# haowenz/FEM

Measured on AMD Instinct MI355X. Metric: mapped Mreads/s (100 bp, e=3) at 1/2/4/8 MI355X + achieved HBM GB/s vs roofline, higher is better.
Workload: dtype u32/u64 integer + 32-bit Myers bit-vectors

## Files before the change

fem_amd/csrc/fem_hip.hip:

```cpp
#include "../../include/fem_hip.h"

#include <hip/hip_runtime.h>
#include <rccl/rccl.h>
#include <sched.h>
#if defined(__x86_64__)
#include <immintrin.h>
#endif

#include <algorithm>
#include <cctype>
#include <cstdio>
#include <cstdlib>
#include <cstring>
#include <condition_variable>
#include <functional>
#include <atomic>
#include <chrono>
#include <mutex>
#include <string>
#include <thread>
#include <vector>

#include "fem_index_build.hip.h"
#include "fem_pack.h"
// ... 476 lines not shown
  hipFuncAttributes a{};
  const bool banked = which == 1;
  const void *f = join ? (const void *)join_kernel(R, which)
                       : banked ? (const void *)femk::seed_select_kernel<R, true> : (const void *)femk::seed_select_kernel<R>;
  return hipFuncGetAttributes(&a, f) == hipSuccess && a.numRegs > 0 ? (uint32_t)a.numRegs : 128u;
}
uint32_t kernel_regs(int R, bool join, int which = 0) {
  static std::atomic<uint32_t> cache[3][2][femk::kMaxR + 1] = {};
  std::atomic<uint32_t> &slot = cache[which][join ? 1 : 0][std::min(std::max(R, 1), femk::kMaxR)];
  uint32_t c = slot.load(std::memory_order_relaxed);
  if (c) return c;
#define FEM_CALL(r) c = kernel_regs_r<r>(join, which)
  FEM_DENSE_SWITCH(R, FEM_CALL)
#undef FEM_CALL
  slot.store(c, std::memory_order_relaxed);
  return c;
}
int select_blocks_per_cu(int R, bool banked, int block, uint32_t lds) {
  int nb = 0;
#define FEM_CALL(r) nb = select_blocks_per_cu_r<r>(banked, block, lds)
  FEM_DENSE_SWITCH(R, FEM_CALL)
#undef FEM_CALL
  return nb;
}
void launch_select(int R, bool banked, dim3 grid, dim3 block, uint32_t lds, hipStream_t st, const femk::SeedParams &sp) {
#define FEM_CALL(r) launch_select_r<r>(banked, grid, block, lds, st, sp)
  FEM_DENSE_SWITCH(R, FEM_CALL)
#undef FEM_CALL
}
int join_blocks_per_cu(int R, int which, int block, uint32_t lds) {
  int nb = 0;
  return hipOccupancyMaxActiveBlocksPerMultiprocessor(&nb, join_kernel(R, which), block, lds) == hipSuccess ? nb : 0;
}
void launch_join(int R, int which, dim3 grid, dim3 block, uint32_t lds, hipStream_t st, const femk::SeedParams &sp) {
  hipLaunchKernelGGL(join_kernel(R, which), grid, block, lds, st, sp);
}

template <int R>
void launch_fast(bool hash, dim3 grid, dim3 block, uint32_t lds, hipStream_t st, const femk::SeedParams &sp) {
  if (hash)
    hipLaunchKernelGGL((femk::seed_fast_kernel<R, true>), grid, block, lds, st, sp);
  else
    hipLaunchKernelGGL((femk::seed_fast_kernel<R, false>), grid, block, lds, st, sp);
}

template <int R>
int fast_blocks_per_cu_r(bool hash, int block, uint32_t lds) {
  int nb = 0;
  hipError_t err = hash ? hipOccupancyMaxActiveBlocksPerMultiprocessor(&nb, femk::seed_fast_kernel<R, true>, block, lds)
                        : hipOccupancyMaxActiveBlocksPerMultiprocessor(&nb, femk::seed_fast_kernel<R, false>, block, lds);
  return err == hipSuccess ? nb : 0;
}
int fast_blocks_per_cu(int R, bool hash, int block, uint32_t lds) {
  switch (R) {
    case 1: return fast_blocks_per_cu_r<1>(hash, block, lds);
    case 2: return fast_blocks_per_cu_r<2>(hash, block, lds);
    case 3: return fast_blocks_per_cu_r<3>(hash, block, lds);
    case 4: return fast_blocks_per_cu_r<4>(hash, block, lds);
    case 5: return fast_blocks_per_cu_r<5>(hash, block, lds);
    case 6: return fast_blocks_per_cu_r<6>(hash, block, lds);
    case 7: return fast_blocks_per_cu_r<7>(hash, block, lds);
    case 8: return fast_blocks_per_cu_r<8>(hash, block, lds);
    case 9: return fast_blocks_per_cu_r<9>(hash, block, lds);
    default: return fast_blocks_per_cu_r<10>(hash, block, lds);
  }
}

// ... 729 lines not shown
  }
  if (!ok_ev) {
    (void)fem_dev_close(h);
    return FEM_ERR_HIP;
  }
  if (testing_switch("FEM_TESTING")) {
    h->no_overlap = testing_switch("FEM_NO_OVERLAP");
    h->no_parts = testing_switch("FEM_NO_PARTS");
    if (const char *mp = getenv("FEM_PARTS")) h->max_parts = std::min(kMaxParts, std::max(1, atoi(mp)));
    h->timeline = testing_switch("FEM_TIMELINE");
    if (h->timeline && hipEventCreate(&h->ev_epoch) == hipSuccess && hipEventRecord(h->ev_epoch, h->side_stream) == hipSuccess)
      h->timing = true, h->have_epoch = true;
    h->force_generic = testing_switch("FEM_FORCE_GENERIC");
    h->force_hash = testing_switch("FEM_FORCE_HASH");
    h->force_dense = testing_switch("FEM_FORCE_DENSE");
    h->no_dense = testing_switch("FEM_NO_DENSE");
    h->no_strided = testing_switch("FEM_NO_STRIDED");
    h->tiny_buffers = testing_switch("FEM_TEST_TINY_BUFFERS");
    if (const char *bl = getenv("FEM_TEST_BANK_BASES")) h->bank_limit = strtoull(bl, nullptr, 10);
    if (const char *bs = getenv("FEM_TEST_BANK_SEQS")) h->bank_seqs = (uint32_t)strtoul(bs, nullptr, 10);
  }
  *out = h;
  return FEM_OK;
}

int fem_dev_close(fem_dev *h) {
  if (!h) return FEM_ERR_INVALID;
  {
    std::lock_guard<std::mutex> lock(g_comm_mu);
    if (g_comm && std::find(g_comm->devs.begin(), g_comm->devs.end(), h->device) != g_comm->devs.end()) destroy_comm_set();
  }
  (void)hipSetDevice(h->device);
  (void)hipDeviceSynchronize();
  delete h->stage_pool;
  h->stage_pool = nullptr;
  for (auto &s : h->slot) {
    drain_timing(h, s);
    for (void *p : {(void *)s.d_bases_alloc, (void *)s.d_off, (void *)s.d_cand, (void *)s.d_meta, (void *)s.d_ed,
                    (void *)s.d_end, (void *)s.d_begin, (void *)s.d_count, (void *)s.d_nmap, (void *)s.d_ctl,
                    (void *)s.d_arena, (void *)s.d_slow, (void *)s.d_sel, (void *)s.d_sel_hdr, (void *)s.d_packed, (void *)s.d_exc_bits, (void *)s.d_quals, (void *)s.d_names,
                    (void *)s.d_name_off, (void *)s.d_count8, (void *)s.d_seg, (void *)s.d_pcand, (void *)s.d_ped, (void *)s.d_pend, (void *)s.d_big})
      if (p) (void)hipFree(p);
    for (void *p : {(void *)s.h_ctl, (void *)s.h_begin, (void *)s.h_count, (void *)s.h_cand, (void *)s.h_ed,
                    (void *)s.h_end, (void *)s.h_bases, (void *)s.h_off, (void *)s.h_quals, (void *)s.h_names, (void *)s.h_name_off,
                    (void *)s.h_count8, (void *)s.h_seg, (void *)s.h_pcand, (void *)s.h_ped, (void *)s.h_pend, (void *)s.h_big})
      if (p) (void)hipHostFree(p);
    if (s.stream) (void)hipStreamDestroy(s.stream);
    if (s.text_stream) (void)hipStreamDestroy(s.text_stream);
    if (s.out_stream) (void)hipStreamDestroy(s.out_stream);
    if (s.ev_text_staged) (void)hipEventDestroy(s.ev_text_staged);
    if (s.ev_text_order) (void)hipEventDestroy(s.ev_text_order);
    delete s.tail;
    s.tail = nullptr;
  }
  delete h->bgzf;
  h->bgzf = nullptr;
  if (h->d_zin) (void)hipFree(h->d_zin);
  if (h->z_stream) (void)hipStreamDestroy(h->z_stream);
  if (h->d_ref_names) (void)hipFree(h->d_ref_names);
  if (h->d_ref_name_off) (void)hipFree(h->d_ref_name_off);
  for (hipEvent_t e : h->event_pool) (void)hipEventDestroy(e);
  if (h->ev_kernels_done) (void)hipEventDestroy(h->ev_kernels_done);
  if (h->ev_select_done) (void)hipEventDestroy(h->ev_select_done);
  if (h->ev_h2d_done) (void)hipEventDestroy(h->ev_h2d_done);
  if (h->ev_epoch) (void)hipEventDestroy(h->ev_epoch);
  if (h->side_stream) (void)hipStreamDestroy(h->side_stream);
// ... 1259 lines not shown
```

fem_amd/csrc/fem_host.cc:

```cpp
#include "fem_host.h"
#include "fem_pack.h"

#include <fcntl.h>
#include <omp.h>
#include <sys/mman.h>
#include <sys/stat.h>
#include <unistd.h>
#include <zlib.h>
#if defined(__x86_64__)
#include <immintrin.h>
#endif

#include <algorithm>
#include <cctype>
#include <cstdio>
#include <cstdlib>
#include <cstring>
#include <condition_variable>
#include <functional>
#include <mutex>
#include <string>
#include <thread>
#include <vector>

namespace {
class SleepingPool {
 public:
  ~SleepingPool() {
    {
      std::lock_guard<std::mutex> l(mu_);
      stop_ = true;
    }
    cv_.notify_all();
    for (auto &t : threads_) t.join();
// ... 2141 lines not shown
    buf.push_back('\n');
    buf.push_back('+');
    buf.push_back('\n');
    buf.insert(buf.end(), qual.begin(), qual.end());
    buf.push_back('\n');
    if (buf.size() > (1u << 24) - 1024) {
      if (fwrite(buf.data(), 1, buf.size(), f) != buf.size()) {
        fclose(f);
        return -2;
      }
      buf.clear();
    }
  }
  bool ok = fwrite(buf.data(), 1, buf.size(), f) == buf.size();
  return (fclose(f) == 0 && ok) ? 0 : -2;
}

int fem_synth_write_fasta(const char *path, const char *text, const uint64_t *seq_off, const uint32_t *seq_len,
                          uint32_t n_seq) {
  FILE *f = fopen(path, "wb");
  if (!f) return -1;
  bool ok = true;
  for (uint32_t s = 0; s < n_seq && ok; ++s) {
    ok = fprintf(f, ">chr%u synthetic\n", s + 1) > 0;
    const char *p = text + seq_off[s];
    for (uint64_t i = 0; i < seq_len[s] && ok; i += 60) {
      size_t n = (size_t)std::min<uint64_t>(60, seq_len[s] - i);
      ok = fwrite(p + i, 1, n, f) == n && fputc('\n', f) != EOF;
    }
  }
  return (fclose(f) == 0 && ok) ? 0 : -2;
}

}
```

fem_amd/csrc/fem_host.h:

```cpp
#ifndef FEM_HOST_H_
#define FEM_HOST_H_

#include <stddef.h>
#include <stdint.h>

#ifdef __cplusplus
extern "C" {
#endif

typedef struct fem_seqfile fem_seqfile;

typedef struct {
  uint64_t n;
  char *bases;
  uint64_t *off;
  char *quals;
  char *names;
  uint64_t *name_off;
} fem_seqset;

fem_seqfile *fem_seqfile_open(const char *path);
void fem_seqfile_close(fem_seqfile *f);
int fem_seqfile_read(fem_seqfile *f, uint64_t max_seqs, fem_seqset *out);
int fem_seqfile_read_bytes(fem_seqfile *f, uint64_t approx_bytes, int n_threads, fem_seqset *out);
// ... 78 lines not shown
  const uint32_t *md_off;
  const char *md;
} fem_record_view;
int fem_records_sam(const fem_tail_ref *ref, const fem_seqset *reads, const fem_record_view *rec, int n_threads,
                    char **text, uint64_t *text_len);
typedef struct {
  uint64_t offset, length;
} fem_text_part;
int fem_records_sam_parts(const fem_tail_ref *ref, const fem_seqset *reads, const fem_record_view *rec, int n_threads,
                          char **buf, uint64_t *cap, fem_text_part *parts, uint64_t *n_asserted);
int fem_records_sam_refs(const fem_tail_ref *ref, const fem_read_refs *reads, const fem_record_view *rec, int n_threads, char **buf,
                         uint64_t *cap, fem_text_part *parts, uint64_t *n_asserted);
int fem_sam_header(const fem_tail_ref *ref, char **text, uint64_t *text_len);
int fem_bam_header(const fem_tail_ref *ref, uint8_t **raw, uint64_t *len);
int fem_sam_fill_quals(char *text, uint64_t text_len, const uint64_t *qual_at, uint64_t n_reads, const char *quals, const uint64_t *off,
                       uint32_t read_len, int n_threads);

void fem_synth_reference(uint64_t seed, uint32_t n_seq, const uint64_t *seq_off, const uint32_t *seq_len, char *out,
                         int n_threads);
void fem_synth_reads(uint64_t seed, const char *ref_text, const uint64_t *seq_off, const uint32_t *seq_len,
                     uint32_t n_seq, uint64_t first_read, uint64_t n_reads, uint32_t L, int32_t e, char *bases_out,
                     int n_threads);
void fem_synth_reads_ex(uint64_t seed, const char *ref_text, const uint64_t *seq_off, const uint32_t *seq_len,
                        uint32_t n_seq, uint64_t first_read, uint64_t n_reads, uint32_t L, int32_t e, char *bases_out,
                        uint8_t *n_err_out, int n_threads);

void fem_synth_reads_packed(uint64_t seed, const char *ref_text, const uint64_t *seq_off, const uint32_t *seq_len, uint32_t n_seq,
                            uint64_t first_read, uint64_t n_reads, uint32_t L, int32_t e, uint8_t *codes, int n_threads);

int fem_synth_write_fastq(const char *path, const char *bases, uint32_t L, uint64_t n_reads, uint64_t first_index);
int fem_synth_write_fasta(const char *path, const char *text, const uint64_t *seq_off, const uint32_t *seq_len,
                          uint32_t n_seq);

#ifdef __cplusplus
}
#endif
#endif
```

fem_amd/csrc/fem_kernels.hip.h:

```cpp
#pragma once
#include <hip/hip_runtime.h>
#include <stdint.h>
#include "fem_planes.hip.h"

namespace femk {

constexpr int kWave = 64;
constexpr uint32_t kFlagCandOverflow = 1u;
constexpr uint32_t kFlagArenaOverflow = 2u;
constexpr uint32_t kFlagTooLarge = 4u;
constexpr uint32_t kInvalidMeta = 0xFFFFFFFFu;
constexpr int kMaxR = 10;
constexpr uint32_t kMeta16 = 0x80000000u;
constexpr uint32_t kSlotChunk = 256u;
constexpr uint32_t kFlagQueueOverflow = 8u;
constexpr uint32_t kQueueChunk = 32u;
constexpr uint32_t kInvalidRead = 0xFFFFFFFFu;

struct SeedLayout {
  uint32_t pkw, nkw;
  uint32_t sf;
  uint32_t dp_rows;
  uint32_t dp_bits;
  uint32_t picked;
// ... 18 lines not shown
  uint32_t *work_cursor;
  const uint32_t *lookup;
  const uint64_t *occ;
  uint32_t inf32;
  const uint32_t *seq_len;
  int32_t e, a, R, k, step, lg;
  uint64_t *cand;
  uint32_t *cand_meta;
  uint32_t cand_cap;
  uint32_t *cand_begin;
  uint32_t *cand_count;
  uint32_t *ctr;
  uint32_t n_seq;
  uint32_t *slow_queue;
  uint32_t slow_cap;
  const uint32_t *work_queue;
  const uint32_t *summary;
  const uint32_t *occ32;
  uint32_t list_shift;
  const uint32_t *goff;
  const uint32_t *blkseq;
  const uint32_t *freq11;
  uint2 *sel;
  uint2 *sel_hdr;
  uint32_t n_banks;
  uint32_t bank_first[5];
  const uint32_t *bank_lo;
  uint32_t n_buckets;
  uint32_t blk_stride;
  unsigned long long *stats;
  uint64_t *arena;
  unsigned long long arena_cap;
  unsigned long long *arena_ctr;
  SeedLayout lay;
};

__global__ void uniform_offsets_kernel(uint64_t *off, uint64_t n, uint32_t len) {
  const uint64_t stride = (uint64_t)gridDim.x * blockDim.x;
  for (uint64_t i = (uint64_t)blockIdx.x * blockDim.x + threadIdx.x; i <= n; i += stride) off[i] = i * (uint64_t)len;
}

__global__ void unpack_reads_kernel(const uint8_t *packed, uint64_t n_reads, uint32_t len, uint32_t bytes_per_read, uint8_t *bases) {
  const uint64_t stride = (uint64_t)gridDim.x * blockDim.x, total = n_reads * bytes_per_read;
  const bool aligned = (len & 3u) == 0u && (((uintptr_t)bases) & 3u) == 0u;
  for (uint64_t i = (uint64_t)blockIdx.x * blockDim.x + threadIdx.x; i < total; i += stride) {
    const uint32_t b = packed[i];
    const uint32_t c0 = (0x54474341u >> (8u * (b & 3u))) & 0xFFu, c1 = (0x54474341u >> (8u * ((b >> 2) & 3u))) & 0xFFu;
    const uint32_t c2 = (0x54474341u >> (8u * ((b >> 4) & 3u))) & 0xFFu, c3 = (0x54474341u >> (8u * (b >> 6))) & 0xFFu;
    if (aligned) {
      ((uint32_t *)bases)[i] = c0 | (c1 << 8) | (c2 << 16) | (c3 << 24);
    } else {
      const uint64_t r = i / bytes_per_read;
      const uint32_t k = (uint32_t)(i - r * bytes_per_read) * 4u;
      uint8_t *o = bases + r * len + k;
      o[0] = (uint8_t)c0;
      if (k + 1u < len) o[1] = (uint8_t)c1;
      if (k + 2u < len) o[2] = (uint8_t)c2;
      if (k + 3u < len) o[3] = (uint8_t)c3;
    }
  }
}
__global__ void scatter_chars_kernel(const uint32_t *at, const uint8_t *ch, uint64_t n, uint8_t *bases) {
  const uint64_t stride = (uint64_t)gridDim.x * blockDim.x;
  for (uint64_t i = (uint64_t)blockIdx.x * blockDim.x + threadIdx.x; i < n; i += stride) bases[at[i]] = ch[i];
}

// ... 1347 lines not shown
```

fem_amd/csrc/fem_seed_join.hip.h:

```cpp
#pragma once
#include "fem_seed_dense.hip.h"

namespace femk {

#ifndef FEM_JOIN_SLOTS_HI
#define FEM_JOIN_SLOTS_HI 32768u
#endif
#ifndef FEM_JOIN_OPT
#define FEM_JOIN_OPT 15
#endif
#ifndef FEM_JOIN_OPT_HI
#define FEM_JOIN_OPT_HI 12
#endif
#ifndef FEM_JOIN_ABL
#define FEM_JOIN_ABL 0
#endif
#ifndef FEM_JOIN_SLOTS_LO
#define FEM_JOIN_SLOTS_LO 32768u
#endif
constexpr uint32_t join_slots(int R, bool padded = false) { return R >= 7 ? FEM_JOIN_SLOTS_HI : padded ? FEM_JOIN_SLOTS_LO : 32768u; }
#ifndef FEM_JOIN_BATCH_HI
#define FEM_JOIN_BATCH_HI 3
#endif

constexpr uint32_t join_bitmap_words(int R, bool padded = false) { return join_slots(R, padded) / 32u + 4u; }

__device__ __forceinline__ void lds_or(uint32_t *w, uint32_t bits) {
  (void)__hip_atomic_fetch_or(w, bits, __ATOMIC_RELAXED, __HIP_MEMORY_SCOPE_WAVEFRONT);
}

template <int R, bool BANKED = false, bool PADDED = false>
__device__ bool join_read(const SeedParams &p, uint32_t s_start, uint32_t s_lo, uint32_t s_freq, uint32_t *bitmap,
                          uint32_t *flg , uint32_t *scatter ,
                          uint32_t *cand_lds, uint32_t &kept0, uint32_t &kept1, uint32_t seq_base = 0u ) {
// ... 441 lines not shown
          const uint32_t fv = ln < nfl ? flg[gg * kFlgStride + ln] : 0u;
          uint32_t rank = 0;
          for (uint64_t m = pm; m;) {
            const int j = __builtin_ctzll(m);
            m &= m - 1;
            const uint32_t x = (uint32_t)__builtin_amdgcn_readlane((int)fv, j);
            rank += (uint32_t)(x < fv || (x == fv && (uint32_t)j < ln));
          }
          wave_sync_lds();
          if (mine) scatter[rank] = fv;
          wave_sync_lds();
          const uint32_t fs = ln < nF ? scatter[ln] : 0u;
          kept = dense_merge_group(cv, kept, fs, nF, e);
          if (kept == 0xFFFFFFFFu) return false;
        }
      }
    }
    cand_lds[(u >= (uint32_t)kStep ? (uint32_t)kWave : 0u) + ln] = cv;
    if (u >= (uint32_t)kStep) kept1 = kept; else kept0 = kept;
    cmin = 0xFFFFFFFFu, cmax = 0u, any_hi = false;
    pm0 = pm1 = pm2 = 0, nf0 = nf1 = nf2 = 0;
  }
  return true;
}

#ifndef FEM_JOIN_WAVES_LO
#define FEM_JOIN_WAVES_LO 7
#endif
#ifndef FEM_JOIN_WAVES_HI
#define FEM_JOIN_WAVES_HI 6
#endif

constexpr int join_waves(int R) { return R <= 6 ? FEM_JOIN_WAVES_LO : FEM_JOIN_WAVES_HI; }

template <int R, bool BANKED = false, bool PADDED = false>
__device__ __forceinline__ void seed_join_body(const SeedParams &p, uint8_t *smem) {
  constexpr uint32_t kSeeds = (uint32_t)(kStep * R);
  static_assert(2 * kStep * R <= kWave, "both strands' seeds must fit the lanes of one wave");
  const uint32_t ln = lane_id();
  const uint32_t wave_in_block = (uint32_t)__builtin_amdgcn_readfirstlane((int)(threadIdx.x >> 6));
  uint8_t *wbase = smem + (size_t)wave_in_block * p.lay.wave_bytes;
  uint32_t *scatter = (uint32_t *)(wbase + p.lay.X);
  uint32_t *flg = (uint32_t *)(wbase + p.lay.A);
  uint32_t *bitmap = (uint32_t *)(wbase + p.lay.F);
  uint2 *blk_entries = (uint2 *)(wbase + p.lay.B);
  uint32_t *cand_lds = (uint32_t *)(wbase + p.lay.sf);
  uint2 *seqtab = (uint2 *)(smem + p.lay.picked);
  const bool small_ref = p.n_seq <= (uint32_t)kWave;
  if (wave_in_block == 0) seqtab[ln] = ln < p.n_seq ? make_uint2(p.goff[ln], p.seq_len[ln]) : make_uint2(0xFFFFFFFFu, 0u);
  __syncthreads();
  for (uint32_t i = ln; i < join_bitmap_words(R, PADDED); i += kWave) bitmap[i] = i < join_slots(R, PADDED) / 32u ? 0u : 0xFFFFFFFFu;
  wave_sync_lds();
  unsigned long long pre_sum = 0, cand_sum = 0;
  SlotChunk chunk, qchunk;

  auto queue_slow = [&](uint32_t read) {
    if (qchunk.left == 0) {
      uint32_t base = 0;
      if (ln == 0) base = atomicAdd(&p.ctr[2], kQueueChunk);
      qchunk.next = bcast0(base);
      qchunk.left = kQueueChunk;
    }
    if (qchunk.next < p.slow_cap) {
      if (ln == 0) p.slow_queue[qchunk.next] = read;
    } else if (ln == 0) {
      atomicOr(&p.ctr[1], kFlagQueueOverflow);
    }
    ++qchunk.next, --qchunk.left;
  };

  for (;;) {
    uint32_t pull = 0;
    if (ln == 0) pull = atomicAdd(p.work_cursor, kReadBlock);
    pull = bcast0(pull);
    if ((uint64_t)p.read_begin + pull >= p.n_reads) break;
    const uint32_t r0 = p.read_begin + pull;
    const uint32_t n_blk = p.n_reads - r0 < kReadBlock ? p.n_reads - r0 : kReadBlock;
    if (ln < 2u * kReadBlock) blk_entries[ln] = make_uint2(kBlkSkip, 0u);
    uint2 hdr = make_uint2(kSelSlow, 0u);
    if (ln < n_blk) hdr = p.sel_hdr[r0 + ln];
    uint2 sel_next = make_uint2(0u, 0u);
    if (!BANKED && ln < 2u * kSeeds) sel_next = p.sel[(size_t)r0 * (2u * kSeeds) + ln];
    for (uint32_t rb = 0; rb < n_blk; ++rb) {
      const uint32_t read = r0 + rb;
      const uint32_t h0 = (uint32_t)__builtin_amdgcn_readlane((int)hdr.x, (int)rb);
      const uint32_t status = h0 & 3u, L = h0 >> 8;
      const uint2 sel = sel_next;
      if (!BANKED && rb + 1u < n_blk && ln < 2u * kSeeds) sel_next = p.sel[(size_t)(read + 1u) * (2u * kSeeds) + ln];
      if (status == kSelSlow) continue;
      if (status == kSelNone) {
        if (ln / 2u == rb) blk_entries[ln] = make_uint2(0u, 0u);
        continue;
      }
      if constexpr (BANKED) {
        constexpr uint32_t kStash = (uint32_t)kWave;
        uint64_t *stash = (uint64_t *)(wbase + p.lay.gq);
        uint32_t acc[2] = {0u, 0u};
        bool failed = false;
        for (uint32_t b = 0; b < p.n_banks && !failed; ++b) {
          uint2 sel_b = make_uint2(0u, 0u);
          if (ln < 2u * kSeeds) sel_b = p.sel[((size_t)read * p.n_banks + b) * (2u * kSeeds) + ln];
          uint32_t kept0 = 0, kept1 = 0;
          if (!join_read<R, true>(p, sel_b.y & 0xFFFFu, sel_b.x, sel_b.y >> 16, bitmap, flg, scatter, cand_lds, kept0, kept1, p.bank_first[b])) {
            failed = true;
            break;
          }
          const uint32_t sq_lo = p.bank_first[b], sq_hi = p.bank_first[b + 1u];
#pragma unroll 1
          for (uint32_t strand = 0; strand < 2u; ++strand) {
            const uint32_t kept = strand ? kept1 : kept0;
            if (kept == 0) continue;
            const uint32_t v = cand_lds[strand * (uint32_t)kWave + ln];
            uint32_t sq = 0, pos = 0, slen = 0;
            if (small_ref) {
              const uint2 tab = seqtab[ln];
              const bool mine = ln >= sq_lo && ln < sq_hi;
              for (uint32_t i = 0; i < kept; ++i) {
                const uint32_t vi = (uint32_t)__builtin_amdgcn_readlane((int)v, (int)i);
                const uint32_t s_i = sq_lo + (uint32_t)__popcll(__builtin_amdgcn_ballot_w64(mine && tab.x <= vi)) - 1u;
                const uint32_t g_i = (uint32_t)__builtin_amdgcn_readlane((int)tab.x, (int)s_i);
                const uint32_t l_i = (uint32_t)__builtin_amdgcn_readlane((int)tab.y, (int)s_i);
                if (ln == i) sq = s_i, pos = vi - g_i, slen = l_i;
              }
            } else if (ln < kept) {
              sq = p.blkseq[(size_t)b * p.blk_stride + (v >> kDenseBlkShift)];
              while (sq + 1u < sq_hi && p.goff[sq + 1u] <= v) ++sq;
              pos = v - p.goff[sq];
              slen = p.seq_len[sq];
            }
            const bool ok = ln < kept && pos >= (uint32_t)p.e && pos + L + (uint32_t)p.e < slen;
            const uint64_t mo = __ballot(ok);
            const uint32_t n_ok = (uint32_t)__popcll(mo);
            if (acc[strand] + n_ok > kStash) {
              failed = true;
              break;
            }
            if (ok) stash[strand * kStash + acc[strand] + (uint32_t)__popcll(mo & ((1ull << ln) - 1ull))] = (((uint64_t)sq << 32) | pos) - (uint64_t)p.e;
            acc[strand] += n_ok;
          }
        }
        if (failed) {
          queue_slow(read);
          continue;
        }
        pre_sum += (uint32_t)__builtin_amdgcn_readlane((int)hdr.y, (int)rb);
        wave_sync_lds();
#pragma unroll 1
        for (uint32_t strand = 0; strand < 2u; ++strand) {
          const uint32_t n_out = acc[strand];
          uint32_t base = 0;
          if (n_out > 0) {
            if (n_out <= chunk.left) {
              base = chunk.next;
              chunk.next += n_out, chunk.left -= n_out;
            } else {
              pad_chunk(p, chunk);
              if (ln == 0) base = atomicAdd(&p.ctr[0], kSlotChunk);
              base = bcast0(base);
              chunk.next = base + n_out, chunk.left = kSlotChunk - n_out;
            }
            if ((unsigned long long)base + n_out > p.cand_cap) {
              if (ln == 0) atomicOr(&p.ctr[1], kFlagCandOverflow);
            } else {
              for (uint32_t i = ln; i < n_out; i += (uint32_t)kWave) {
                p.cand[base + i] = stash[strand * kStash + i];
                p.cand_meta[base + i] = (read * 2u + strand) | (i < (n_out & ~7u) ? kMeta16 : 0u);
              }
            }
          }
          if (ln == 0) blk_entries[2u * rb + strand] = make_uint2(base, n_out);
          cand_sum += n_out;
        }
        wave_sync_lds();
        continue;
      }
      const uint32_t s_lo = sel.x, s_start = sel.y & 0xFFFFu, s_freq = sel.y >> 16;
      uint32_t kept0 = 0, kept1 = 0;
      if (!join_read<R, false, PADDED>(p, s_start, s_lo, s_freq, bitmap, flg, scatter, cand_lds, kept0, kept1)) {
        queue_slow(read);
        continue;
      }
      if (FEM_JOIN_ABL & 16) kept0 = kept1 = 0;
      pre_sum += (uint32_t)__builtin_amdgcn_readlane((int)hdr.y, (int)rb);
#pragma unroll 1
      for (uint32_t strand = 0; strand < 2u; ++strand) {
        const uint32_t kept = strand ? kept1 : kept0;
        uint64_t out = 0;
        bool ok = false;
        if (kept == 0) {
          if (ln == 0) blk_entries[2u * rb + strand] = make_uint2(0u, 0u);
          continue;
        }
        const uint32_t v = cand_lds[strand * (uint32_t)kWave + ln];
        uint32_t sq = 0, pos = 0, slen = 0;
        if (small_ref) {
          const uint2 tab = seqtab[ln];
          for (uint32_t i = 0; i < kept; ++i) {
            const uint32_t vi = (uint32_t)__builtin_amdgcn_readlane((int)v, (int)i);
            const uint32_t s_i = (uint32_t)__popcll(__builtin_amdgcn_ballot_w64(tab.x <= vi)) - 1u;
            const uint32_t g_i = (uint32_t)__builtin_amdgcn_readlane((int)tab.x, (int)s_i);
            const uint32_t l_i = (uint32_t)__builtin_amdgcn_readlane((int)tab.y, (int)s_i);
            if (ln == i) sq = s_i, pos = vi - g_i, slen = l_i;
          }
        } else if (ln < kept) {
          sq = p.blkseq[v >> kDenseBlkShift];
          while (sq + 1u < p.n_seq && p.goff[sq + 1u] <= v) ++sq;
          pos = v - p.goff[sq];
          slen = p.seq_len[sq];
        }
        if (ln < kept) {
          ok = pos >= (uint32_t)p.e && pos + L + (uint32_t)p.e < slen;
          out = (((uint64_t)sq << 32) | pos) - (uint64_t)p.e;
        }
        const uint64_t mo = __ballot(ok);
        const uint32_t n_out = (uint32_t)__popcll(mo);
        uint32_t base = 0;
        if (n_out > 0) {
          if (n_out <= chunk.left) {
            base = chunk.next;
            chunk.next += n_out, chunk.left -= n_out;
          } else {
            pad_chunk(p, chunk);
            if (ln == 0) base = atomicAdd(&p.ctr[0], kSlotChunk);
            base = bcast0(base);
            chunk.next = base + n_out, chunk.left = kSlotChunk - n_out;
          }
          if ((unsigned long long)base + n_out > p.cand_cap) {
            if (ln == 0) atomicOr(&p.ctr[1], kFlagCandOverflow);
          } else if (ok) {
            const uint32_t rank = (uint32_t)__popcll(mo & ((1ull << ln) - 1ull)), at = base + rank;
            p.cand[at] = out;
            p.cand_meta[at] = (read * 2u + strand) | (rank < (n_out & ~7u) ? kMeta16 : 0u);
          }
        }
        if (ln == 0) blk_entries[2u * rb + strand] = make_uint2(base, n_out);
        cand_sum += n_out;
      }
    }
    wave_sync_lds();
    const uint2 entry = blk_entries[ln];
    wave_sync_lds();
    if (ln < 2u * kReadBlock && r0 + ln / 2u < p.n_reads && entry.x != kBlkSkip) {
      __builtin_nontemporal_store(entry.x, &p.cand_begin[r0 * 2u + ln]);
      __builtin_nontemporal_store(entry.y, &p.cand_count[r0 * 2u + ln]);
    }
  }
  pad_chunk(p, chunk);
  for (uint32_t i = ln; i < qchunk.left; i += kWave)
    if (qchunk.next + i < p.slow_cap) p.slow_queue[qchunk.next + i] = kInvalidRead;
  if (ln == 0) {
    if (pre_sum) atomicAdd(&p.stats[0], pre_sum);
    if (cand_sum) atomicAdd(&p.stats[1], cand_sum);
  }
}


#define FEM_JOIN_KERNEL(R, WAVES)                                                                                               \
  __global__ void __launch_bounds__(256) __attribute__((amdgpu_waves_per_eu(WAVES, 8))) seed_join_kernel_r##R(SeedParams p) {                         \
    extern __shared__ __attribute__((aligned(16))) uint8_t smem[];                                                               \
    seed_join_body<R>(p, smem);                                                                                                  \
  }                                                                                                                              \
  __global__ void __launch_bounds__(256) __attribute__((amdgpu_waves_per_eu(FEM_JOIN_WAVES_HI, 8))) seed_join_banked_kernel_r##R(SeedParams p) {  \
    extern __shared__ __attribute__((aligned(16))) uint8_t smem[];                                                               \
    seed_join_body<R, true>(p, smem);                                                                                            \
  }                                                                                                                              \
  __global__ void __launch_bounds__(256) __attribute__((amdgpu_waves_per_eu(WAVES, 8))) seed_join_kernel_padded_r##R(SeedParams p) {  \
    extern __shared__ __attribute__((aligned(16))) uint8_t smem[];                                                               \
    seed_join_body<R, false, true>(p, smem);                                                                                     \
  }
FEM_JOIN_KERNEL(1, FEM_JOIN_WAVES_LO)
FEM_JOIN_KERNEL(2, FEM_JOIN_WAVES_LO)
FEM_JOIN_KERNEL(3, FEM_JOIN_WAVES_LO)
FEM_JOIN_KERNEL(4, FEM_JOIN_WAVES_LO)
FEM_JOIN_KERNEL(5, FEM_JOIN_WAVES_LO)
FEM_JOIN_KERNEL(6, FEM_JOIN_WAVES_LO)
FEM_JOIN_KERNEL(7, FEM_JOIN_WAVES_HI)
FEM_JOIN_KERNEL(8, FEM_JOIN_WAVES_HI)
FEM_JOIN_KERNEL(9, FEM_JOIN_WAVES_HI)
FEM_JOIN_KERNEL(10, FEM_JOIN_WAVES_HI)
// ... 4 lines not shown
```

fem_amd/csrc/fem_seed_select.hip.h:

```cpp
#pragma once
#include <type_traits>

#include "fem_seed_fast.hip.h"

namespace femk {

constexpr uint32_t kDenseMaxBanks = 4;
constexpr uint32_t kDenseNear = 1024u;
constexpr uint32_t kDenseRemap = 0xF0000000u;
constexpr uint32_t kSelKeepAll = 1u << 15;
constexpr uint32_t kSelOk = 0u, kSelNone = 1u, kSelSlow = 2u;
constexpr uint32_t kSelMaxCols = 128u;
constexpr uint32_t kSelMaxList = 128u;
constexpr uint32_t kX11 = 1u << 22;

__device__ __forceinline__ uint32_t wave_min_u32(uint32_t x) {
  constexpr uint32_t kFill = 0xFFFFFFFFu;
  x = dpp_min_step<0x111, 0xF>(x, kFill), x = dpp_min_step<0x112, 0xF>(x, kFill), x = dpp_min_step<0x114, 0xF>(x, kFill);
  x = dpp_min_step<0x118, 0xF>(x, kFill), x = dpp_min_step<0x142, 0xA>(x, kFill), x = dpp_min_step<0x143, 0xC>(x, kFill);
  return (uint32_t)__builtin_amdgcn_readlane((int)x, 63);
}
__device__ __forceinline__ uint32_t wave_max_u32(uint32_t x) {
  return (uint32_t)__builtin_amdgcn_readlane((int)wave_scan_max(x), 63);
}
// ... 87 lines not shown

template <int R, bool BANKED = false>
__global__ void __launch_bounds__(256) __attribute__((amdgpu_waves_per_eu(FEM_SELECT_WAVES, 8))) seed_select_kernel(SeedParams p) {
  extern __shared__ __attribute__((aligned(16))) uint8_t smem[];
  const uint32_t ln = lane_id();
  const uint32_t wave_in_block = (uint32_t)__builtin_amdgcn_readfirstlane((int)(threadIdx.x >> 6));
  uint8_t *wbase = smem + (size_t)wave_in_block * p.lay.wave_bytes;
  uint64_t *boff = (uint64_t *)(wbase + p.lay.rb);
  uint32_t *fw = (uint32_t *)(wbase + p.lay.strm);
  uint32_t *nw = fw + p.lay.strm_words;
  uint16_t *fq = (uint16_t *)(wbase + p.lay.fq);
  uint32_t *r_base = (uint32_t *)(wbase + p.lay.rinfo), *r_len = r_base + kReadBlock, *r_flag = r_len + kReadBlock,
           *r_pre = r_flag + kReadBlock;
  constexpr uint32_t kOk0 = 1u, kOk1 = 2u, kShape = 4u, kSlow = 8u;
  const uint32_t sstride = p.lay.gstride, nb = p.lay.nb;
  const uint32_t inf = p.inf32;
  SlotChunk qchunk;

  auto queue_slow = [&](uint32_t read) {
    if (qchunk.left == 0) {
      uint32_t base = 0;
      if (ln == 0) base = atomicAdd(&p.ctr[2], kQueueChunk);
      qchunk.next = bcast0(base);
      qchunk.left = kQueueChunk;
    }
    if (qchunk.next < p.slow_cap) {
      if (ln == 0) p.slow_queue[qchunk.next] = read;
    } else if (ln == 0) {
      atomicOr(&p.ctr[1], kFlagQueueOverflow);
    }
    ++qchunk.next, --qchunk.left;
  };

  for (;;) {
    uint32_t pull = 0;
    if (ln == 0) pull = atomicAdd(p.work_cursor, kReadBlock);
    pull = bcast0(pull);
    if ((uint64_t)p.read_begin + pull >= p.n_reads) break;
    const uint32_t r0 = p.read_begin + pull;
    const uint32_t n_blk = p.n_reads - r0 < kReadBlock ? p.n_reads - r0 : kReadBlock;
    wave_sync_lds();
    if (ln <= n_blk) boff[ln] = p.read_off[r0 + ln];
    wave_sync_lds();
    for (uint32_t sb = 0; sb < n_blk; sb += nb) {
      const uint32_t cnt = n_blk - sb < nb ? n_blk - sb : nb;
      const uint32_t rd0 = r0 + sb;
      const uint64_t o_first = boff[sb];
      const uint64_t blk_off = (uint64_t)__builtin_amdgcn_readfirstlane((uint32_t)o_first) |
                               ((uint64_t)__builtin_amdgcn_readfirstlane((uint32_t)(o_first >> 32)) << 32);
      uint32_t my_S = 0, my_flag = 0;
      {
        uint32_t L = 0, base = 0;
        if (ln < cnt) {
          const uint64_t o0 = boff[sb + ln], o1 = boff[sb + ln + 1u];
          L = (uint32_t)(o1 - o0), base = (uint32_t)(o0 - blk_off);
          const int S = (int)L - kK + 1;
          bool shape_ok = S > 0 && R <= S / kStep;
          if (shape_ok) shape_ok = (S - (kStep - 1)) / kStep - R * kLg + 2 >= 2;
          if (shape_ok) {
            my_S = (uint32_t)S;
            my_flag = kShape | kOk0 | kOk1;
            const uint32_t widest = (uint32_t)(S / kStep - R * kLg + 1);
            if (widest > kSelMaxCols || p.a == 0) my_flag |= kSlow;
          }
        }
        if (ln < kReadBlock) r_base[ln] = base, r_len[ln] = L, r_flag[ln] = my_flag, r_pre[ln] = 0;
      }
      const uint32_t total_chars = (uint32_t)(boff[sb + cnt] - blk_off);
      uint32_t any_n = 0;
      {
        const uint8_t *src = p.bases + blk_off;
// ... 238 lines not shown
```

fem_amd/host.py:

```python
import ctypes as C
import os

import numpy as np

_HERE = os.path.dirname(os.path.abspath(__file__))
_LIB = None


class SeqSet(C.Structure):
    _fields_ = [("n", C.c_uint64), ("bases", C.c_void_p), ("off", C.c_void_p), ("quals", C.c_void_p),
                ("names", C.c_void_p), ("name_off", C.c_void_p)]


class TailInput(C.Structure):
    _fields_ = [("n_reads", C.c_uint64), ("cand_begin", C.c_void_p), ("cand_count", C.c_void_p), ("cand", C.c_void_p),
                ("ed", C.c_void_p), ("end", C.c_void_p)]


class TailRef(C.Structure):
    _fields_ = [("text", C.c_void_p), ("off", C.c_void_p), ("len", C.c_void_p), ("n_seq", C.c_uint32),
                ("names", C.c_void_p), ("name_off", C.c_void_p)]


class Records(C.Structure):
# ... 32 lines not shown
        L.fem_seqfile_open.restype = vp
        L.fem_seqfile_open.argtypes = [C.c_char_p]
        L.fem_seqfile_close.argtypes = [vp]
        L.fem_seqfile_read.argtypes = [vp, u64, C.POINTER(SeqSet)]
        L.fem_seqset_free.argtypes = [C.POINTER(SeqSet)]
        L.fem_seqfile_read_bytes.argtypes = [vp, u64, C.c_int, C.POINTER(SeqSet)]
        L.fem_seqfile_plan.argtypes = [vp, u64, C.c_int, C.POINTER(vp), C.POINTER(BatchShape)]
        L.fem_seqfile_plan_count.argtypes = [vp, u64, C.c_int, C.POINTER(vp), C.POINTER(BatchShape)]
        L.fem_seqfile_fill.argtypes = [vp, vp, C.c_int, vp, vp, vp, vp, vp]
        L.fem_seqfile_fill_packed.argtypes = [vp, vp, C.c_int, C.c_uint32, vp, u64, C.POINTER(u64), vp, vp, vp]
        L.fem_seqfile_fill_packed_refs.argtypes = [vp, vp, C.c_int, C.c_uint32, vp, u64, C.POINTER(u64), vp]
        L.fem_batch_plan_free.argtypes = [vp]
        L.fem_records_sam.argtypes = [C.POINTER(TailRef), C.POINTER(SeqSet), C.POINTER(RecordView), C.c_int, C.POINTER(vp),
                                      C.POINTER(u64)]
        L.fem_records_sam_parts.argtypes = [C.POINTER(TailRef), C.POINTER(SeqSet), C.POINTER(RecordView), C.c_int,
                                            C.POINTER(vp), C.POINTER(u64), C.POINTER(TextPart), C.POINTER(u64)]
        L.fem_index_save.argtypes = [C.c_char_p, i32, i32, vp, u64, vp]
        L.fem_index_load.argtypes = [C.c_char_p, C.POINTER(i32), C.POINTER(i32), C.POINTER(vp), C.POINTER(u64),
                                     C.POINTER(vp)]
        L.fem_tail_records.argtypes = [i32, C.POINTER(TailRef), vp, vp, C.POINTER(TailInput), C.c_int,
                                       C.POINTER(Records)]
        L.fem_records_free.argtypes = [C.POINTER(Records)]
        L.fem_tail_sam.argtypes = [i32, C.POINTER(TailRef), C.POINTER(SeqSet), C.POINTER(TailInput), C.c_int,
                                   C.POINTER(vp), C.POINTER(u64)]
        L.fem_sam_header.argtypes = [C.POINTER(TailRef), C.POINTER(vp), C.POINTER(u64)]
        L.fem_bam_header.argtypes = [C.POINTER(TailRef), C.POINTER(vp), C.POINTER(u64)]
        L.fem_sam_fill_quals.argtypes = [vp, u64, vp, u64, vp, vp, C.c_uint32, C.c_int]
        L.fem_synth_reference.argtypes = [u64, C.c_uint32, vp, vp, vp, C.c_int]
        L.fem_synth_reads.argtypes = [u64, vp, vp, vp, C.c_uint32, u64, u64, C.c_uint32, i32, vp, C.c_int]
        L.fem_synth_reads_ex.argtypes = [u64, vp, vp, vp, C.c_uint32, u64, u64, C.c_uint32, i32, vp, vp, C.c_int]
        L.fem_synth_reads_packed.argtypes = [u64, vp, vp, vp, C.c_uint32, u64, u64, C.c_uint32, i32, vp, C.c_int]
        L.fem_synth_write_fastq.argtypes = [C.c_char_p, vp, C.c_uint32, u64, u64]
        L.fem_synth_write_fasta.argtypes = [C.c_char_p, vp, vp, vp, C.c_uint32]
        L.free = C.CDLL(None).free
        L.free.argtypes = [vp]
        _LIB = L
    return _LIB


def _copy(ptr, n, dtype):
    n = int(n)
    if n == 0 or not ptr:
        return np.zeros(0, dtype=dtype)
    buf = (C.c_char * (n * np.dtype(dtype).itemsize)).from_address(ptr)
    return np.frombuffer(buf, dtype=dtype, count=n).copy()


def synth_reference(seed, seq_lens, threads=8):
    lens = np.asarray(seq_lens, dtype=np.uint32)
    off = np.zeros(len(lens), dtype=np.uint64)
    if len(lens) > 1:
        off[1:] = np.cumsum(lens[:-1], dtype=np.uint64)
    total = int(lens.astype(np.uint64).sum())
    text = np.zeros(total + 64, dtype=np.uint8)
    lib().fem_synth_reference(seed, len(lens), off.ctypes.data, lens.ctypes.data, text.ctypes.data, threads)
    return text, off, lens


def synth_reads(seed, text, off, lens, n_reads, L, e, first_read=0, threads=8, out=None, out_offsets=None, n_err=None):
    bases = np.zeros(n_reads * L + 8, dtype=np.uint8) if out is None else out
    assert bases.dtype == np.uint8 and len(bases) >= n_reads * L
    ne = 0
    if n_err is not None:
        assert n_err.dtype == np.uint8 and len(n_err) >= n_reads
        ne = n_err.ctypes.data
    lib().fem_synth_reads_ex(seed, text.ctypes.data, off.ctypes.data, lens.ctypes.data, len(lens), first_read, n_reads,
                             L, e, bases.ctypes.data, ne, threads)
    if out_offsets is None:
        offsets = np.arange(n_reads + 1, dtype=np.uint64) * np.uint64(L)
    else:
        offsets = out_offsets
        offsets[:n_reads + 1] = np.arange(n_reads + 1, dtype=np.uint64) * np.uint64(L)
    return bases, offsets


def synth_reads_packed(seed, text, off, lens, n_reads, L, e, out, first_read=0, threads=8):
    bpr = (L + 3) // 4
    assert out.dtype == np.uint8 and len(out) >= ((n_reads * bpr + 7) & ~7)
    lib().fem_synth_reads_packed(seed, text.ctypes.data, off.ctypes.data, lens.ctypes.data, len(lens), first_read, n_reads,
                                 L, e, out.ctypes.data, threads)
    return out


def write_fastq(path, bases, L, n_reads, first_index=0):
    rc = lib().fem_synth_write_fastq(path.encode(), bases.ctypes.data, L, n_reads, first_index)
    if rc != 0:
        raise OSError("fem_synth_write_fastq failed (%d)" % rc)


def write_fasta(path, text, off, lens):
    rc = lib().fem_synth_write_fasta(path.encode(), text.ctypes.data, off.ctypes.data, lens.ctypes.data, len(lens))
    if rc != 0:
        raise OSError("fem_synth_write_fasta failed (%d)" % rc)


class Sequences:

    def __init__(self, s):
        n = int(s.n)
        self.n = n
        self.off = _copy(s.off, n + 1, np.uint64)
        self.name_off = _copy(s.name_off, n + 1, np.uint64)
        nb = int(self.off[-1]) if n else 0
        self.bases = _copy(s.bases, nb, np.uint8)
        self.quals = _copy(s.quals, nb, np.uint8) if s.quals else None
        self.names_raw = _copy(s.names, int(self.name_off[-1]) if n else 0, np.uint8)

    def seq(self, i):
        return self.bases[int(self.off[i]):int(self.off[i + 1])].tobytes()

    def name(self, i):
        return self.names_raw[int(self.name_off[i]):int(self.name_off[i + 1])].tobytes().decode()

    def qual(self, i):
        return self.quals[int(self.off[i]):int(self.off[i + 1])].tobytes()


def read_sequences(path, max_seqs=0):
    L = lib()
    f = L.fem_seqfile_open(path.encode())
    if not f:
        raise FileNotFoundError(path)
    s = SeqSet()
    rc = L.fem_seqfile_read(f, max_seqs, C.byref(s))
    L.fem_seqfile_close(f)
    try:
# ... 348 lines not shown
```

Before: 336.8.

## Schedule join work with guided tickets, prefetch next block, and static first pull

Replaces the join kernel's fixed-size atomic read-block pulls with a ticket scheme. Blocks of 16 reads shrink to 8/4/2/1 near the tail to balance the end of the launch. The first ticket is assigned statically, and the next ticket is drawn and its headers prefetched one read before the current block ends, to hide atomic and load latency. The select kernel also gets a static first pull, and candidate slot chunks grow to fit large outputs. Optional timestamp instrumentation and host ticket helpers are added for testing, at the cost of more complex scheduling logic.

After: 320.2. -4.9%, worse.

```diff
diff --git a/fem_amd/csrc/fem_hip.hip b/fem_amd/csrc/fem_hip.hip
--- a/fem_amd/csrc/fem_hip.hip
+++ b/fem_amd/csrc/fem_hip.hip
@@ -532,7 +532,44 @@
   int nb = 0;
   return hipOccupancyMaxActiveBlocksPerMultiprocessor(&nb, join_kernel(R, which), block, lds) == hipSuccess ? nb : 0;
 }
+#ifdef FEM_JOIN_STAMPS
+constexpr uint32_t kStampLaunches = 32, kStampWaves = 16384;
+struct StampRing {
+  unsigned long long *d = nullptr;
+  uint64_t launches = 0;
+  uint64_t waves[kStampLaunches], reads[kStampLaunches];
+} g_stamps;
+unsigned long long *stamps_next(uint32_t waves, uint32_t reads) {
+  if (!g_stamps.d && hipMalloc((void **)&g_stamps.d, sizeof(unsigned long long) * 4u * kStampWaves * kStampLaunches) != hipSuccess) return nullptr;
+  if (waves > kStampWaves) return nullptr;
+  const uint32_t at = (uint32_t)(g_stamps.launches++ % kStampLaunches);
+  g_stamps.waves[at] = waves, g_stamps.reads[at] = reads;
+  return g_stamps.d + (size_t)at * 4u * kStampWaves;
+}
+void stamps_dump() {
+  if (!g_stamps.d || !g_stamps.launches) return;
+  const char *path = getenv("FEM_JOIN_STAMPS_OUT");
+  FILE *f = fopen(path ? path : "join_stamps.bin", "wb");
+  const uint64_t n = std::min<uint64_t>(g_stamps.launches, kStampLaunches);
+  std::vector<unsigned long long> buf(4u * kStampWaves);
+  for (uint64_t i = 0; f && i < n; ++i) {
+    const uint32_t at = (uint32_t)((g_stamps.launches - n + i) % kStampLaunches);
+    if (hipMemcpy(buf.data(), g_stamps.d + (size_t)at * 4u * kStampWaves, sizeof(unsigned long long) * 4u * g_stamps.waves[at], hipMemcpyDeviceToHost) != hipSuccess) break;
+    const unsigned long long head[2] = {g_stamps.waves[at], g_stamps.reads[at]};
+    fwrite(head, sizeof(head), 1, f);
+    fwrite(buf.data(), sizeof(unsigned long long), 4u * g_stamps.waves[at], f);
+  }
+  if (f) fclose(f);
+  g_stamps.launches = 0;
+}
+#endif
 void launch_join(int R, int which, dim3 grid, dim3 block, uint32_t lds, hipStream_t st, const femk::SeedParams &sp) {
+#ifdef FEM_JOIN_STAMPS
+  femk::SeedParams stamped = sp;
+  stamped.stamps = stamps_next(grid.x * (block.x / 64u), sp.n_reads - sp.read_begin);
+  hipLaunchKernelGGL(join_kernel(R, which), grid, block, lds, st, stamped);
+  return;
+#endif
   hipLaunchKernelGGL(join_kernel(R, which), grid, block, lds, st, sp);
 }
 
@@ -1328,6 +1365,9 @@
   }
   (void)hipSetDevice(h->device);
   (void)hipDeviceSynchronize();
+#ifdef FEM_JOIN_STAMPS
+  stamps_dump();
+#endif
   delete h->stage_pool;
   h->stage_pool = nullptr;
   for (auto &s : h->slot) {
diff --git a/fem_amd/csrc/fem_host.cc b/fem_amd/csrc/fem_host.cc
--- a/fem_amd/csrc/fem_host.cc
+++ b/fem_amd/csrc/fem_host.cc
@@ -1,5 +1,6 @@
 #include "fem_host.h"
 #include "fem_pack.h"
+#include "fem_ticket.h"
 
 #include <fcntl.h>
 #include <omp.h>
@@ -2207,4 +2208,17 @@
   return (fclose(f) == 0 && ok) ? 0 : -2;
 }
 
-}
+uint32_t fem_join_ticket_block(uint32_t t, uint32_t n, uint32_t waves, uint32_t *out) {
+  const femticket::Block b = femticket::block_of(t, n, waves);
+  if (out) out[0] = b.first, out[1] = b.count;
+  return femticket::ticket_count(n, waves);
+}
+uint32_t fem_join_ticket_blocks(uint32_t n, uint32_t waves, uint32_t *first, uint32_t *count, uint32_t cap) {
+  for (uint32_t t = 0; t < cap; ++t) {
+    const femticket::Block b = femticket::block_of(t, n, waves);
+    first[t] = b.first, count[t] = b.count;
+  }
+  return femticket::ticket_count(n, waves);
+}
+
+}
diff --git a/fem_amd/csrc/fem_host.h b/fem_amd/csrc/fem_host.h
--- a/fem_amd/csrc/fem_host.h
+++ b/fem_amd/csrc/fem_host.h
@@ -134,6 +134,9 @@
 int fem_synth_write_fasta(const char *path, const char *text, const uint64_t *seq_off, const uint32_t *seq_len,
                           uint32_t n_seq);
 
+uint32_t fem_join_ticket_block(uint32_t t, uint32_t n, uint32_t waves, uint32_t *out);
+uint32_t fem_join_ticket_blocks(uint32_t n, uint32_t waves, uint32_t *first, uint32_t *count, uint32_t cap);
+
 #ifdef __cplusplus
 }
 #endif
diff --git a/fem_amd/csrc/fem_kernels.hip.h b/fem_amd/csrc/fem_kernels.hip.h
--- a/fem_amd/csrc/fem_kernels.hip.h
+++ b/fem_amd/csrc/fem_kernels.hip.h
@@ -74,6 +74,9 @@
   uint64_t *arena;
   unsigned long long arena_cap;
   unsigned long long *arena_ctr;
+#ifdef FEM_JOIN_STAMPS
+  unsigned long long *stamps;
+#endif
   SeedLayout lay;
 };
 
diff --git a/fem_amd/csrc/fem_seed_join.hip.h b/fem_amd/csrc/fem_seed_join.hip.h
--- a/fem_amd/csrc/fem_seed_join.hip.h
+++ b/fem_amd/csrc/fem_seed_join.hip.h
@@ -1,5 +1,6 @@
 #pragma once
 #include "fem_seed_dense.hip.h"
+#include "fem_ticket.h"
 
 namespace femk {
 
@@ -507,6 +508,13 @@
 #endif
 
 constexpr int join_waves(int R) { return R <= 6 ? FEM_JOIN_WAVES_LO : FEM_JOIN_WAVES_HI; }
+#ifndef FEM_JOIN_SLOT_CHUNK
+#define FEM_JOIN_SLOT_CHUNK 32
+#endif
+constexpr uint32_t kJoinSlotChunk = FEM_JOIN_SLOT_CHUNK;
+#ifndef FEM_JOIN_SCHED
+#define FEM_JOIN_SCHED 3
+#endif
 
 template <int R, bool BANKED = false, bool PADDED = false>
 __device__ __forceinline__ void seed_join_body(const SeedParams &p, uint8_t *smem) {
@@ -528,6 +536,10 @@
   wave_sync_lds();
   unsigned long long pre_sum = 0, cand_sum = 0;
   SlotChunk chunk, qchunk;
+#ifdef FEM_JOIN_STAMPS
+  const uint64_t st_entry = __builtin_amdgcn_s_memrealtime();
+  uint64_t st_first = 0, st_last = st_entry, st_pull = 0;
+#endif
 
   auto queue_slow = [&](uint32_t read) {
     if (qchunk.left == 0) {
@@ -544,24 +556,65 @@
     ++qchunk.next, --qchunk.left;
   };
 
-  for (;;) {
-    uint32_t pull = 0;
-    if (ln == 0) pull = atomicAdd(p.work_cursor, kReadBlock);
-    pull = bcast0(pull);
-    if ((uint64_t)p.read_begin + pull >= p.n_reads) break;
-    const uint32_t r0 = p.read_begin + pull;
-    const uint32_t n_blk = p.n_reads - r0 < kReadBlock ? p.n_reads - r0 : kReadBlock;
+  auto block_of_ticket = [&](uint32_t t_wave, bool drawn) -> femticket::Block {
+    uint32_t grid = gridDim.x;
+    asm volatile("" : "+s"(grid));
+    const uint32_t waves = grid * (blockDim.x >> 6);
+    return femticket::block_of(drawn && (FEM_JOIN_SCHED & 1) ? t_wave + waves : t_wave, p.n_reads - p.read_begin, waves);
+  };
+  uint32_t first_ticket = blockIdx.x * (blockDim.x >> 6) + wave_in_block;
+  if (!(FEM_JOIN_SCHED & 1)) {
+    if (ln == 0) first_ticket = atomicInc(p.work_cursor, 0xFFFFFFFFu);
+    first_ticket = bcast0(first_ticket);
+  }
+  femticket::Block cur = block_of_ticket(first_ticket, false);
+  uint2 hdr = make_uint2(kSelSlow, 0u);
+  uint2 sel_next = make_uint2(0u, 0u);
+#ifdef FEM_JOIN_STAMPS
+  uint64_t st_t0 = __builtin_amdgcn_s_memrealtime();
+#endif
+  if (ln < cur.count) hdr = p.sel_hdr[p.read_begin + cur.first + ln];
+  if (!BANKED && cur.count != 0u && ln < 2u * kSeeds) sel_next = p.sel[(size_t)(p.read_begin + cur.first) * (2u * kSeeds) + ln];
+  while (cur.count != 0u) {
+    const uint32_t r0 = p.read_begin + cur.first, n_blk = cur.count;
     if (ln < 2u * kReadBlock) blk_entries[ln] = make_uint2(kBlkSkip, 0u);
-    uint2 hdr = make_uint2(kSelSlow, 0u);
-    if (ln < n_blk) hdr = p.sel_hdr[r0 + ln];
-    uint2 sel_next = make_uint2(0u, 0u);
-    if (!BANKED && ln < 2u * kSeeds) sel_next = p.sel[(size_t)r0 * (2u * kSeeds) + ln];
+#ifdef FEM_JOIN_STAMPS
+    {
+      asm volatile("" ::"v"(hdr.x), "v"(hdr.y), "v"(sel_next.x), "v"(sel_next.y));
+      const uint64_t now = __builtin_amdgcn_s_memrealtime();
+      st_pull += now - st_t0;
+      if (st_first == 0) st_first = now;
+    }
+#endif
     for (uint32_t rb = 0; rb < n_blk; ++rb) {
       const uint32_t read = r0 + rb;
       const uint32_t h0 = (uint32_t)__builtin_amdgcn_readlane((int)hdr.x, (int)rb);
+      const uint32_t pre = (uint32_t)__builtin_amdgcn_readlane((int)hdr.y, (int)rb);
       const uint32_t status = h0 & 3u, L = h0 >> 8;
       const uint2 sel = sel_next;
-      if (!BANKED && rb + 1u < n_blk && ln < 2u * kSeeds) sel_next = p.sel[(size_t)(read + 1u) * (2u * kSeeds) + ln];
+      if ((FEM_JOIN_SCHED & 2) && n_blk == 1u) {
+        if (ln == 63u) hdr.x = atomicInc(p.work_cursor, 0xFFFFFFFFu);
+      }
+      uint32_t sel_of = read + 1u;
+      bool sel_any = rb + 1u < n_blk;
+      if ((FEM_JOIN_SCHED & 2) && rb + 1u == n_blk) {
+#ifdef FEM_JOIN_STAMPS
+        const uint64_t st_a = __builtin_amdgcn_s_memrealtime();
+#endif
+        const uint32_t drawn = (uint32_t)__builtin_amdgcn_readlane((int)hdr.x, 63);
+#ifdef FEM_JOIN_STAMPS
+        st_pull += __builtin_amdgcn_s_memrealtime() - st_a;
+#endif
+        const femticket::Block nxt = block_of_ticket(drawn, true);
+        sel_of = p.read_begin + nxt.first, sel_any = nxt.count != 0u;
+        if (!BANKED && sel_any && ln < 2u * kSeeds) sel_next = p.sel[(size_t)sel_of * (2u * kSeeds) + ln];
+        if (ln < nxt.count) hdr = p.sel_hdr[p.read_begin + nxt.first + ln];
+      } else {
+        if (!BANKED && sel_any && ln < 2u * kSeeds) sel_next = p.sel[(size_t)sel_of * (2u * kSeeds) + ln];
+      }
+      if ((FEM_JOIN_SCHED & 2) && rb + 2u == n_blk) {
+        if (ln == 63u) hdr.x = atomicInc(p.work_cursor, 0xFFFFFFFFu);
+      }
       if (status == kSelSlow) continue;
       if (status == kSelNone) {
         if (ln / 2u == rb) blk_entries[ln] = make_uint2(0u, 0u);
@@ -618,7 +671,7 @@
           queue_slow(read);
           continue;
         }
-        pre_sum += (uint32_t)__builtin_amdgcn_readlane((int)hdr.y, (int)rb);
+        pre_sum += pre;
         wave_sync_lds();
 #pragma unroll 1
         for (uint32_t strand = 0; strand < 2u; ++strand) {
@@ -630,9 +683,10 @@
               chunk.next += n_out, chunk.left -= n_out;
             } else {
               pad_chunk(p, chunk);
-              if (ln == 0) base = atomicAdd(&p.ctr[0], kSlotChunk);
+              const uint32_t want = n_out > kJoinSlotChunk ? n_out : kJoinSlotChunk;
+              if (ln == 0) base = atomicAdd(&p.ctr[0], want);
               base = bcast0(base);
-              chunk.next = base + n_out, chunk.left = kSlotChunk - n_out;
+              chunk.next = base + n_out, chunk.left = want - n_out;
             }
             if ((unsigned long long)base + n_out > p.cand_cap) {
               if (ln == 0) atomicOr(&p.ctr[1], kFlagCandOverflow);
@@ -656,7 +710,7 @@
         continue;
       }
       if (FEM_JOIN_ABL & 16) kept0 = kept1 = 0;
-      pre_sum += (uint32_t)__builtin_amdgcn_readlane((int)hdr.y, (int)rb);
+      pre_sum += pre;
 #pragma unroll 1
       for (uint32_t strand = 0; strand < 2u; ++strand) {
         const uint32_t kept = strand ? kept1 : kept0;
@@ -696,9 +750,10 @@
             chunk.next += n_out, chunk.left -= n_out;
           } else {
             pad_chunk(p, chunk);
-            if (ln == 0) base = atomicAdd(&p.ctr[0], kSlotChunk);
+            const uint32_t want = n_out > kJoinSlotChunk ? n_out : kJoinSlotChunk;
+            if (ln == 0) base = atomicAdd(&p.ctr[0], want);
             base = bcast0(base);
-            chunk.next = base + n_out, chunk.left = kSlotChunk - n_out;
+            chunk.next = base + n_out, chunk.left = want - n_out;
           }
           if ((unsigned long long)base + n_out > p.cand_cap) {
             if (ln == 0) atomicOr(&p.ctr[1], kFlagCandOverflow);
@@ -719,7 +774,25 @@
       __builtin_nontemporal_store(entry.x, &p.cand_begin[r0 * 2u + ln]);
       __builtin_nontemporal_store(entry.y, &p.cand_count[r0 * 2u + ln]);
     }
+#ifdef FEM_JOIN_STAMPS
+    st_last = st_t0 = __builtin_amdgcn_s_memrealtime();
+#endif
+    if (!(FEM_JOIN_SCHED & 2)) {
+      uint32_t drawn = 0;
+      if (ln == 0) drawn = atomicInc(p.work_cursor, 0xFFFFFFFFu);
+      cur = block_of_ticket(bcast0(drawn), true);
+      if (ln < cur.count) hdr = p.sel_hdr[p.read_begin + cur.first + ln];
+      if (!BANKED && cur.count != 0u && ln < 2u * kSeeds) sel_next = p.sel[(size_t)(p.read_begin + cur.first) * (2u * kSeeds) + ln];
+    } else {
+      cur = block_of_ticket((uint32_t)__builtin_amdgcn_readlane((int)hdr.x, 63), true);
+    }
   }
+#ifdef FEM_JOIN_STAMPS
+  if (p.stamps && ln == 0) {
+    unsigned long long *o = p.stamps + 4u * (size_t)(blockIdx.x * (blockDim.x >> 6) + wave_in_block);
+    o[0] = st_entry, o[1] = st_first ? st_first : st_entry, o[2] = st_last, o[3] = st_pull;
+  }
+#endif
   pad_chunk(p, chunk);
   for (uint32_t i = ln; i < qchunk.left; i += kWave)
     if (qchunk.next + i < p.slow_cap) p.slow_queue[qchunk.next + i] = kInvalidRead;
diff --git a/fem_amd/csrc/fem_seed_select.hip.h b/fem_amd/csrc/fem_seed_select.hip.h
--- a/fem_amd/csrc/fem_seed_select.hip.h
+++ b/fem_amd/csrc/fem_seed_select.hip.h
@@ -143,11 +143,13 @@
     ++qchunk.next, --qchunk.left;
   };
 
-  for (;;) {
-    uint32_t pull = 0;
-    if (ln == 0) pull = atomicAdd(p.work_cursor, kReadBlock);
-    pull = bcast0(pull);
-    if ((uint64_t)p.read_begin + pull >= p.n_reads) break;
+  const uint32_t waves = gridDim.x * (blockDim.x >> 6);
+  auto next_pull = [&]() -> uint32_t {
+    uint32_t at = 0;
+    if (ln == 0) at = atomicAdd(p.work_cursor, kReadBlock);
+    return bcast0(at) + waves * kReadBlock;
+  };
+  for (uint32_t pull = (blockIdx.x * (blockDim.x >> 6) + wave_in_block) * kReadBlock; (uint64_t)p.read_begin + pull < p.n_reads; pull = next_pull()) {
     const uint32_t r0 = p.read_begin + pull;
     const uint32_t n_blk = p.n_reads - r0 < kReadBlock ? p.n_reads - r0 : kReadBlock;
     wave_sync_lds();
diff --git a/fem_amd/csrc/fem_ticket.h b/fem_amd/csrc/fem_ticket.h
--- /dev/null
+++ b/fem_amd/csrc/fem_ticket.h
@@ -0,0 +1,56 @@
+#pragma once
+#include <stdint.h>
+
+#if defined(__HIPCC__)
+#define FEM_TICKET_FN __host__ __device__ inline
+#else
+#define FEM_TICKET_FN inline
+#endif
+
+namespace femticket {
+
+#ifndef FEM_JOIN_TAIL
+#define FEM_JOIN_TAIL 1
+#endif
+constexpr uint32_t kTail8 = FEM_JOIN_TAIL ? 8u : 0u, kTail4 = FEM_JOIN_TAIL ? 4u : 0u, kTail2 = FEM_JOIN_TAIL ? 2u : 0u,
+                   kTail1 = FEM_JOIN_TAIL ? 2u : 0u;
+
+struct Block {
+  uint32_t first, count;
+};
+
+FEM_TICKET_FN uint32_t umin(uint32_t a, uint32_t b) { return a < b ? a : b; }
+
+FEM_TICKET_FN Block block_of(uint32_t t, uint32_t n, uint32_t W) {
+  const uint32_t n1 = umin(n, kTail1 * W);
+  const uint32_t n2 = umin(n - n1, kTail2 * W);
+  const uint32_t n4 = umin(n - n1 - n2, kTail4 * W);
+  const uint32_t n8 = umin(n - n1 - n2 - n4, kTail8 * W);
+  const uint32_t n16 = n - n1 - n2 - n4 - n8;
+  uint32_t begin = 0, len = n16, size = 16u;
+  uint32_t blocks = (n16 + 15u) >> 4;
+  if (t >= blocks) t -= blocks, begin += len, len = n8, size = 8u, blocks = (n8 + 7u) >> 3;
+  if (size == 8u && t >= blocks) t -= blocks, begin += len, len = n4, size = 4u, blocks = (n4 + 3u) >> 2;
+  if (size == 4u && t >= blocks) t -= blocks, begin += len, len = n2, size = 2u, blocks = (n2 + 1u) >> 1;
+  if (size == 2u && t >= blocks) t -= blocks, begin += len, len = n1, size = 1u, blocks = n1;
+  Block b;
+  if (t >= blocks) {
+    b.first = n, b.count = 0u;
+    return b;
+  }
+  const uint32_t at = t * size;
+  b.first = begin + at;
+  b.count = umin(size, len - at);
+  return b;
+}
+
+FEM_TICKET_FN uint32_t ticket_count(uint32_t n, uint32_t W) {
+  const uint32_t n1 = umin(n, kTail1 * W);
+  const uint32_t n2 = umin(n - n1, kTail2 * W);
+  const uint32_t n4 = umin(n - n1 - n2, kTail4 * W);
+  const uint32_t n8 = umin(n - n1 - n2 - n4, kTail8 * W);
+  const uint32_t n16 = n - n1 - n2 - n4 - n8;
+  return ((n16 + 15u) >> 4) + ((n8 + 7u) >> 3) + ((n4 + 3u) >> 2) + ((n2 + 1u) >> 1) + n1;
+}
+
+}
diff --git a/fem_amd/host.py b/fem_amd/host.py
--- a/fem_amd/host.py
+++ b/fem_amd/host.py
@@ -88,6 +88,10 @@
         L.fem_synth_reads_packed.argtypes = [u64, vp, vp, vp, C.c_uint32, u64, u64, C.c_uint32, i32, vp, C.c_int]
         L.fem_synth_write_fastq.argtypes = [C.c_char_p, vp, C.c_uint32, u64, u64]
         L.fem_synth_write_fasta.argtypes = [C.c_char_p, vp, vp, vp, C.c_uint32]
+        L.fem_join_ticket_block.restype = C.c_uint32
+        L.fem_join_ticket_block.argtypes = [C.c_uint32, C.c_uint32, C.c_uint32, vp]
+        L.fem_join_ticket_blocks.restype = C.c_uint32
+        L.fem_join_ticket_blocks.argtypes = [C.c_uint32, C.c_uint32, vp, vp, C.c_uint32]
         L.free = C.CDLL(None).free
         L.free.argtypes = [vp]
         _LIB = L
@@ -148,6 +152,15 @@
     rc = lib().fem_synth_write_fasta(path.encode(), text.ctypes.data, off.ctypes.data, lens.ctypes.data, len(lens))
     if rc != 0:
         raise OSError("fem_synth_write_fasta failed (%d)" % rc)
+
+
+def join_ticket_blocks(n, waves, extra=4):
+    total = int(lib().fem_join_ticket_block(0, n, waves, None))
+    cap = total + extra
+    first, count = np.zeros(cap, np.uint32), np.zeros(cap, np.uint32)
+    got = int(lib().fem_join_ticket_blocks(n, waves, first.ctypes.data, count.ctypes.data, cap))
+    assert got == total
+    return first, count, total
 
 
 class Sequences:
```
